# pytorch/ao

Measured on AMD Instinct MI355X. Metric: linear-layer tokens/sec, Llama-3-8B int4-wo (tinygemm g128), bs=1, higher is better.
Workload: dtype bf16 x int4 (dequant bf16, fp32 accumulate); 1 GPU; Int4WeightOnlyConfig(group_size=128) Llama-3-8B linear shapes, bs=1 seq=1, 32 layers x {qkv 6144x4096, o 4096x4096, gate 14336x4096, up 14336x4096, down 4096x14336}; module_layout=SURVEY.md 8(d) five shapes (qkv merged; gate, up separate), launch=hipGraph replay, parallelism=dp1 (one token stream per GPU, no collective)

## Files before the change

ao_amd/_lib.py:

```python
import ctypes
import os
import re
import threading

_HERE = os.path.dirname(os.path.abspath(__file__))
LIB_PATH = os.environ.get("AO_MI355_LIB") or os.path.join(_HERE, "_C_mi355.so")
HEADER_PATH = os.path.join(os.path.dirname(_HERE), "include", "ao_mi355.h")

AO_OK = 0
AO_ERR_INVALID_ARGUMENT = -1
AO_ERR_NULL_POINTER = -2
AO_ERR_HIP = -3

_lock = threading.Lock()
_lib = None

_P = ctypes.c_void_p
_I64 = ctypes.c_int64
_INT = ctypes.c_int

_SIGNATURES = {
    "ao_abi_version": [],
    "ao_prof_enable": [_INT],
    "ao_prof_collect": [_P, _INT, _P],
    "ao_splitk_reserve": [_P, _I64],
    "ao_splitk_query": [_P, _P],
    "ao_int4_convert_weight_to_int4pack": [_P, _P, _I64, _I64, _INT, _P],
    "ao_int4_unpack_int4pack": [_P, _P, _I64, _I64, _INT, _P],
    "ao_int4_weight_int4pack_mm": [_P, _P, _P, _P, _I64, _I64, _I64, _INT, _P],
    "ao_int4_weight_int4pack_mm_pair": [_P, _P, _P, _P, _P, _P, _P, _P, _I64, _I64, _I64, _INT, _P],
    "ao_int4_pair_independent": [_P, _P, _P, _P, _I64, _I64, _I64],
    "ao_int4_pair_fusions": [],
    "ao_int4_dequantize": [_P, _P, _P, _I64, _I64, _INT, _P],
    "ao_int4_quantize_tinygemm": [_P, _P, _P, _I64, _I64, _INT, _P],
    "ao_int4_hqq_workspace_bytes": [_I64, _I64, _INT],
    "ao_int4_quantize_hqq": [_P, _P, _P, _P, _I64, _I64, _INT, _P],
    "ao_int4_plain_quantize": [_P, _P, _P, _P, _I64, _I64, _INT, _INT, _P],
    "ao_int4_set_tuning": [_INT, _INT],
    "ao_int4_set_trace": [_P],
    "ao_gemm8_set_variant": [_INT],
    "ao_gemm8_set_tuning": [_INT, _INT],
    "ao_int4_mm_kernel_name": [_I64, _I64, _I64, _INT],
    "ao_gemm8_kernel_name": [_INT, _I64, _I64, _I64],
    "ao_fp8_int4_kernel_name": [_I64, _I64, _I64, _INT],
    "ao_gemm8_plan": [_INT, _I64, _I64, _I64, _P, _P],
    "ao_gemm8_plan_rows": [_INT, _I64, _I64, _I64, _P],
    "ao_gemm8_route": [_INT, _I64, _I64, _I64, _INT, _P, _INT],
# ... 157 lines not shown
            l.ao_fp8_block_grouped_mm_kernel_name.restype = ctypes.c_char_p
        if hasattr(l, "ao_nvfp4_linear_kernel_name"):
            l.ao_nvfp4_linear_kernel_name.restype = ctypes.c_char_p
        if hasattr(l, "ao_nvfp4_grouped_mm_kernel_name"):
            l.ao_nvfp4_grouped_mm_kernel_name.restype = ctypes.c_char_p
        if hasattr(l, "ao_fp8_int4_kernel_name"):
            l.ao_fp8_int4_kernel_name.restype = ctypes.c_char_p
        l.ao_moe_padded_rows.restype = _I64
        l.ao_mx_blocked_rows.restype = _I64
        l.ao_allreduce_flag_bytes.restype = _I64
        l.ao_allreduce_state_bytes.restype = _I64
        if hasattr(l, "ao_moe_a2a_flag_bytes"):
            l.ao_moe_a2a_flag_bytes.restype = _I64
            l.ao_moe_a2a_state_bytes.restype = _I64
        l.ao_int4_hqq_workspace_bytes.restype = _I64
        _lib = l
    return _lib


def last_error():
    return lib().ao_last_error().decode("utf-8", "replace")


def check(rc):
    if rc == AO_OK:
        return
    msg = last_error()
    if rc == AO_ERR_INVALID_ARGUMENT:
        raise ValueError(msg)
    raise RuntimeError(msg)
# ... 1 lines not shown
```

ao_amd/csrc/int4_kernels.hip:

```cpp
#include <algorithm>
#include <mutex>
#include <type_traits>
#include <utility>

#include "common.h"
#include "lds_dma.h"
#include "splitk.h"

namespace ao {
void fp8_rowwise_rb_set_trace(unsigned long long* p);
namespace {

__device__ __forceinline__ void dequant_word(uint32_t p, float s, float neg8s, float z,
                                             uint32_t (&out)[4]) {
  uint32_t lo = p & 0x0F0F0F0Fu;
  uint32_t hi = (p >> 4) & 0x0F0F0F0Fu;
  asm("" : "+v"(lo));
  asm("" : "+v"(hi));
  const float f0 = (float)(lo & 0xffu), f4 = (float)((lo >> 8) & 0xffu);
  const float f1 = (float)((lo >> 16) & 0xffu), f5 = (float)(lo >> 24);
  const float f2 = (float)(hi & 0xffu), f6 = (float)((hi >> 8) & 0xffu);
  const float f3 = (float)((hi >> 16) & 0xffu), f7 = (float)(hi >> 24);
  const f32x2 q[4] = {{f0, f1}, {f2, f3}, {f4, f5}, {f6, f7}};
#pragma unroll
// ... 68 lines not shown
    d.w0 = widen_add(ident, d.tp0, d.tp1, zz);
    d.w1 = widen_add(ident, d.tp2, d.tp3, zz);
#endif
  } else {
    d.out[0] = pack_bf16x2(d.w0.x, d.w0.y); d.out[1] = pack_bf16x2(d.w0.z, d.w0.w);
    d.out[2] = pack_bf16x2(d.w1.x, d.w1.y); d.out[3] = pack_bf16x2(d.w1.z, d.w1.w);
  }
}

template <int MAXM>
struct XRegs {
  static constexpr int kDwords = (MAXM <= 4) ? MAXM : MAXM;
  uint32_t v[kDwords];
};

template <int G, int MAXM, int DEPTH, bool STRAIGHT, bool BAL, bool STAMP>
__device__ __forceinline__ void int4_mm_body(
    const uint16_t* __restrict__ x, const u32x4* __restrict__ qdata,
    const uint32_t* __restrict__ sz, uint16_t* __restrict__ y, int M, int N, int K, float* __restrict__ ws, unsigned* __restrict__ tickets,
    const unsigned bx, const unsigned nbx) {
  static_assert(!(BAL || STAMP) || (STRAIGHT && MAXM == 1 && DEPTH == 4), "the balanced grid and the stamps exist on the 8 x 4 straight-line form");
  unsigned long long stamp[6] = {0, 0, 0, 0, 0, 0};
  if constexpr (STAMP) { stamp[0] = __builtin_amdgcn_s_memrealtime(); stamp[2] = __builtin_amdgcn_s_memtime(); }
  constexpr int NG = (G >= 128) ? 1 : (128 / G);
  constexpr int ROWSTRIDE = (MAXM <= 4) ? 256 : 272;
  constexpr int SLAB = (MAXM + 1) * ROWSTRIDE;
  extern __shared__ __attribute__((aligned(16))) char smem[];

  const int lane = threadIdx.x & 63;
  const int wave = __builtin_amdgcn_readfirstlane(threadIdx.x >> 6);
  const int nwaves = blockDim.x >> 6;
  int ntile = (int)bx;
  int kwave = wave;
  int part = -1;
  const int halves = BAL ? 2 * ((int)nbx - (N >> 4)) : 0;
  if constexpr (BAL) {
// ... 62 lines not shown
      }
    } else {
#pragma unroll
      for (int i = 0; i < MAXM / 4; ++i) {
        const int rr = min((lane >> 4) + 4 * i, last_row);
        const u32x4 t = *reinterpret_cast<const u32x4*>(xrow0 + (size_t)rr * K + kb * 128 + (lane & 15) * 8);
        s.xr.v[4 * i + 0] = t.x; s.xr.v[4 * i + 1] = t.y;
        s.xr.v[4 * i + 2] = t.z; s.xr.v[4 * i + 3] = t.w;
      }
    }
  };

  f32x4 acc = {0.f, 0.f, 0.f, 0.f};
  const s16x4 ident = identity_fragment(lane);

  auto stage_x = [&](const Stage& s, char* dst) {
    if (MAXM <= 4) {
#pragma unroll
      for (int r = 0; r < MAXM; ++r)
        *reinterpret_cast<uint32_t*>(dst + r * ROWSTRIDE + st_off) = s.xr.v[r];
    } else {
#pragma unroll
      for (int i = 0; i < MAXM / 4; ++i) {
        const int r = (lane >> 4) + 4 * i;
        char* d = dst + r * ROWSTRIDE + st_off;
        *reinterpret_cast<u32x2*>(d) = u32x2{s.xr.v[4 * i + 0], s.xr.v[4 * i + 1]};
        *reinterpret_cast<u32x2*>(d + 64) = u32x2{s.xr.v[4 * i + 2], s.xr.v[4 * i + 3]};
      }
    }
  };
// ... 19 lines not shown
    }
  };

  const int kb_last = max(kb1 - 1, kb0);
#pragma unroll
  for (int d = 0; d < DEPTH; ++d) issue(st[d], kFixedRun ? kb0 + d : min(kb0 + d, kb_last));

  auto for_slots = [&](auto&& f) {
    [&]<int... D>(std::integer_sequence<int, D...>) { (f(std::integral_constant<int, D>{}), ...); }(std::make_integer_sequence<int, DEPTH>{});
  };
  if constexpr (STRAIGHT) {
    if constexpr (STAMP) {
      asm volatile("s_waitcnt vmcnt(%0)" ::"n"(NG + 1 + (DEPTH - 1) * (NG + 2)) : "memory");
      stamp[3] = __builtin_amdgcn_s_memtime();
    }
    for_slots([&](auto dc) {
      constexpr int d = decltype(dc)::value;
      consume(st[d]);
    });
    if constexpr (STAMP) {
      asm volatile("" ::"v"(acc));
      stamp[4] = __builtin_amdgcn_s_memtime();
    }
    float* r = red + wave * 256 + (kq * 4) * 16 + (lane & 15);
    r[0] = acc.x; r[16] = acc.y; r[32] = acc.z; r[48] = acc.w;
    acc = f32x4{0.f, 0.f, 0.f, 0.f};
  } else {
  int kb = kb0;
  for (; kb + 2 * DEPTH <= kb1; kb += DEPTH) {
    for_slots([&](auto dc) {
      constexpr int d = decltype(dc)::value;
      consume(st[d]);
// ... 49 lines not shown
          if (t == 1u) __hip_atomic_store(&tickets[pair], 0u, __ATOMIC_RELAXED, __HIP_MEMORY_SCOPE_AGENT);
        }
        t = __builtin_amdgcn_readfirstlane(t);
        if (t == 1u && lane < 16) {
          float other[4];
#pragma unroll
          for (int w = 0; w < 4; ++w)
            other[w] = __builtin_bit_cast(float, __builtin_amdgcn_raw_buffer_load_b32(rws, ((1 - part) * 64 + w * 16 + lane) * 4, 0, kSc1));
          float sum = 0.f;
#pragma unroll
          for (int w = 0; w < 8; ++w) sum += ((w >> 2) == part) ? red[(w & 3) * 256 + lane] : other[w & 3];
          y[(size_t)ntile * 16 + lane] = f32_to_bf16_bits(sum);
        }
      }
      write_stamps();
      return;
    }
  }
  const int row = tid >> 4, col = tid & 15;
  if (tid < 256 && row < rows) {
    float sum = 0.f;
    for (int w = 0; w < nwaves; ++w) sum += red[w * 256 + tid];
    y[(size_t)(m0 + row) * N + ntile * 16 + col] = f32_to_bf16_bits(sum);
  }
  write_stamps();
}

template <int G, int MAXM, int DEPTH, bool STRAIGHT = false, bool BAL = false, bool STAMP = false>
__global__ __launch_bounds__((MAXM > 4) ? 512 : 1024) void int4_mm_kernel(
    const uint16_t* __restrict__ x, const u32x4* __restrict__ qdata,
    const uint32_t* __restrict__ sz, uint16_t* __restrict__ y, int M, int N, int K, float* __restrict__ ws, unsigned* __restrict__ tickets) {
  int4_mm_body<G, MAXM, DEPTH, STRAIGHT, BAL, STAMP>(x, qdata, sz, y, M, N, K, ws, tickets, blockIdx.x, gridDim.x);
}

struct Int4PairArgs {
  const uint16_t* x0; const uint16_t* x1;
  const u32x4* q0; const u32x4* q1;
  const uint32_t* sz0; const uint32_t* sz1;
  uint16_t* y0; uint16_t* y1;
  int N, K;
  float* ws;
  unsigned* tickets;
};
template <int G, int DEPTH, bool BAL>
__global__ __launch_bounds__(1024) void int4_mm_pair_kernel(const Int4PairArgs a) {
  const bool second = blockIdx.z != 0;
  const int halves = BAL ? (int)gridDim.x - (a.N >> 4) : 0;
  int4_mm_body<G, 1, DEPTH, true, BAL, false>(second ? a.x1 : a.x0, second ? a.q1 : a.q0, second ? a.sz1 : a.sz0, second ? a.y1 : a.y0, 1, a.N, a.K,
                                              a.ws + (second ? (size_t)halves * 128 : 0), a.tickets + (second ? halves : 0), blockIdx.x, gridDim.x);
}

constexpr int kRbStages = 3;
constexpr int kRbWeightStages = 3;
constexpr int rb_wstages(int waves, int mt, int wst) {
  const int room = (160 * 1024 - kRbStages * mt * 4096) / (waves * wst);
  return room >= kRbWeightStages ? kRbWeightStages : (room < 3 ? 3 : room);
}

template <int G, int WAVES, int NT, int MT = 8, int ABL = 0, bool PROD = false>
__global__ __launch_bounds__(64 * WAVES * (PROD ? 2 : 1), (WAVES == 4 && !PROD) ? 2 : 1) void int4_mm_rb_kernel(
    const uint16_t* __restrict__ x, const u32x4* __restrict__ qdata, const uint32_t* __restrict__ sz, uint16_t* __restrict__ y, int M,
    int N, int K, float* __restrict__ ws, unsigned* __restrict__ tickets, unsigned long long* __restrict__ trace) {
  unsigned long long ts[13] = {0, 0, 0, 0, 0, 0, 0, 0, 0, 0, 0, 0, 0};
  if (ABL == 5) ts[0] = __builtin_amdgcn_s_memtime();
// ... 886 lines not shown
  }
  std::lock_guard<std::mutex> lock(mu);
  if (cached[dev] == 0) {
    int n = 0;
    if (hipDeviceGetAttribute(&n, hipDeviceAttributeMultiprocessorCount, dev) != hipSuccess || n <= 0) {
      (void)hipGetLastError();
      n = 256;
    }
    cached[dev] = n;
  }
  return cached[dev];
}

constexpr int kBalOff = 981, kBalOn = 982, kStampGrid = 983, kStampBal = 984;
constexpr int kPairOff = 985, kPairHalves = 986;

Int4Route int4_route(int64_t M, int64_t N, int64_t K, int G, const Int4Force& f) {
  Int4Route r;
  const bool bal_mode = (f.mode >= kBalOff && f.mode <= kStampBal) || f.mode == kPairOff || f.mode == kPairHalves;
  if (f.mode != 0 && !bal_mode) r = int4_forced_route(M, N, K, G, f);
  else if (M <= 16 && !(M > 8 && (N >> 4) >= 288) && !(M > 4 && (N >> 4) >= 1024)) r = tile_route(M, N, K);
  else if (w32_band(M, N)) r = w32_route(M, N, K, G);
  else r = rb_route(M, N, K, (M <= 16) ? 1 : (M <= 32) ? 2 : (M <= 64) ? 4 : 8);
  r.wpb = f.wpb;
  if ((f.mode == 0 || bal_mode) && r.form == Int4Route::Tile && r.rows == 1 && r.straight && r.depth == 4 && (K >> 7) == 32) {
    const bool forced = f.mode == kBalOn || f.mode == kStampBal;
    if (f.mode != kBalOff && f.mode != kStampGrid) r.halves = ao_int4_balanced_halves(N >> 4, device_cus(), forced);
    r.stamp = (f.mode == kStampGrid || f.mode == kStampBal) && G == 128;
  }
  return r;
}

#define AO_MM_ARGS x, qdata, sz, y, M, N, K

template <int G>
int launch_route(const Int4Route& r, const uint16_t* x, const int32_t* qdata, const uint16_t* sz, uint16_t* y, int64_t M, int64_t N, int64_t K,
                 hipStream_t stream) {
  const int s = r.split;
  switch (r.form) {
// ... 157 lines not shown

int launch_pair(int group_size, const PairGeom& g, const Int4Problem& a, const Int4Problem& b, int64_t N, int64_t K, hipStream_t stream) {
  float* ws = nullptr;
  unsigned* tickets = nullptr;
  if (g.halves > 0)
    if (int rc = splitk_workspace(stream, &ws, &tickets, (size_t)2 * g.halves * 128, 2)) return rc;
  const Int4PairArgs args = pair_args(a, b, N, K, ws, tickets);
  return with_pair_kernel(group_size, g.depth, g.halves > 0, [&](auto kern) {
    if (int rc = ensure_dynamic_lds(reinterpret_cast<const void*>(kern), g.smem, "hipFuncSetAttribute(int4_mm_pair_kernel)")) return rc;
    ao::launch(kern, g.grid, g.block, g.smem, stream, args);
    AO_LAUNCH_CHECK("int4_mm_pair_kernel launch");
    return (int)AO_OK;
  });
}

struct Capture {
  bool active = false;
  unsigned long long id = 0;
  const hipGraphNode_t* deps = nullptr;
  size_t ndeps = 0;
};
Capture capture_of(hipStream_t s) {
  Capture c;
  hipStreamCaptureStatus st = hipStreamCaptureStatusNone;
  hipGraph_t graph = nullptr;
  if (hipStreamGetCaptureInfo_v2(s, &st, &c.id, &graph, &c.deps, &c.ndeps) != hipSuccess) {
    (void)hipGetLastError();
    return Capture{};
  }
  c.active = st == hipStreamCaptureStatusActive;
  return c;
}

struct PairRecord {
  bool live = false, paired = false;
  unsigned long long id = 0;
  hipStream_t stream = nullptr;
  hipGraphNode_t node = nullptr;
  int group_size = 0, depth = 0, halves = 0;
  int64_t N = 0, K = 0;
  Int4Problem p{};
};
std::mutex g_pair_mu;
PairRecord g_pair;
long long g_pair_fusions = 0;

bool try_fuse_pair(const Capture& cap, hipStream_t stream, const Int4Route& r, int group_size, int64_t N, int64_t K, const Int4Problem& b, bool keep_halves) {
  std::lock_guard<std::mutex> lock(g_pair_mu);
  PairRecord& rec = g_pair;
  if (!rec.live) return false;
  if (rec.id != cap.id) {
    rec = PairRecord{};
    return false;
  }
  if (rec.paired || rec.stream != stream || cap.ndeps != 1 || cap.deps == nullptr || cap.deps[0] != rec.node) return false;
  if (rec.group_size != group_size || rec.N != N || rec.K != K || rec.depth != r.depth || rec.halves != r.halves) return false;
  if (!ao_int4_pair_independent(rec.p.x, rec.p.y, b.x, b.y, 1, N, K)) return false;
  PairGeom g;
  if (!pair_geometry(r, 1, N, K, keep_halves, &g)) return false;
  float* ws = nullptr;
  unsigned* tickets = nullptr;
  if (g.halves > 0 && !splitk_workspace_held(stream, &ws, &tickets, (size_t)2 * g.halves * 128)) return false;
  Int4PairArgs args = pair_args(rec.p, b, N, K, ws, tickets);
  const hipGraphNode_t node = rec.node;
  const int rc = with_pair_kernel(group_size, g.depth, g.halves > 0, [&](auto kern) {
    void* params[1] = {&args};
    hipKernelNodeParams np{};
    np.func = reinterpret_cast<void*>(kern);
    np.gridDim = g.grid;
    np.blockDim = g.block;
    np.sharedMemBytes = (unsigned)g.smem;
    np.kernelParams = params;
    np.extra = nullptr;
    const hipError_t e = hipGraphKernelNodeSetParams(node, &np);
    if (e != hipSuccess) {
      (void)hipGetLastError();
      set_error("int4 pair fusion: hipGraphKernelNodeSetParams refused the pair kernel: %s (%s); launched on its own", hipGetErrorString(e), hipGetErrorName(e));
      return (int)AO_ERR_HIP;
    }
    return (int)AO_OK;
  });
  if (rc != AO_OK) {
    rec = PairRecord{};
    return false;
  }
  rec.paired = true;
  ++g_pair_fusions;
  return true;
}

void record_pair_candidate(const Capture& before, hipStream_t stream, const Int4Route& r, int group_size, int64_t N, int64_t K, const Int4Problem& p) {
  const Capture now = capture_of(stream);
  hipGraphNodeType type = hipGraphNodeTypeCount;
  const bool ok = now.active && now.id == before.id && now.ndeps == 1 && now.deps != nullptr &&
                  hipGraphNodeGetType(now.deps[0], &type) == hipSuccess && type == hipGraphNodeTypeKernel;
  if (!ok) (void)hipGetLastError();
  std::lock_guard<std::mutex> lock(g_pair_mu);
  g_pair = PairRecord{};
  if (!ok) return;
  g_pair.live = true;
  g_pair.id = now.id;
  g_pair.stream = stream;
  g_pair.node = now.deps[0];
  g_pair.group_size = group_size; g_pair.depth = r.depth; g_pair.halves = r.halves;
  g_pair.N = N; g_pair.K = K;
  g_pair.p = p;
}

}
}

using namespace ao;

extern "C" int ao_int4_balanced_halves(int64_t tiles, int cus, int forced) {
  if (tiles <= 0 || cus <= 0) return 0;
  const int64_t r = tiles % cus;
  if (r > kSplitMaxTickets) return 0;
  if (forced) return (int)r;
  return (tiles > cus && tiles <= 4ll * cus && 2 * r == cus) ? (int)r : 0;
}

// ... 69 lines not shown
extern "C" int ao_int4_weight_int4pack_mm(const uint16_t* x, const int32_t* qdata,
                                          const uint16_t* scale_and_zero, uint16_t* y, int64_t M,
                                          int64_t N, int64_t K, int group_size, void* stream) {
  AO_REQUIRE_PTR(qdata);
  AO_REQUIRE_PTR(scale_and_zero);
  if (int rc = check_int4_shape(__func__, N, K, group_size)) return rc;
  AO_REQUIRE(M >= 0 && M < (1ll << 31), "ao_int4_weight_int4pack_mm: bad M=%lld", (long long)M);
  if (M == 0) return AO_OK;
  AO_REQUIRE_PTR(x);
  AO_REQUIRE_PTR(y);
  hipStream_t s = (hipStream_t)stream;
  Capture cap;
  Int4Route twin;
  bool candidate = false;
  const Int4Problem prob{x, qdata, scale_and_zero, y};
  if (M == 1 && (cap = capture_of(s)).active) {
    PairGeom g;
    twin = int4_route(M, N, K, group_size, g_int4_force);
    candidate = pair_geometry(twin, M, N, K, true, &g);
    if (candidate && g_int4_force.mode != kPairOff && try_fuse_pair(cap, s, twin, group_size, N, K, prob, g_int4_force.mode == kPairHalves))
      return AO_OK;
  }
  const int64_t by_bytes = ((1ll << 32) - 1) / (2 * K) / 128 * 128;
  const int64_t chunk = std::max<int64_t>(128, std::min<int64_t>(by_bytes, 65535ll * 16));
  for (int64_t m0 = 0; m0 < M; m0 += chunk) {
    const int64_t rows = std::min(chunk, M - m0);
    const uint16_t* xc = x + m0 * K;
    uint16_t* yc = y + m0 * N;
    int rc;
    switch (group_size) {
      case 32: rc = dispatch_mm<32>(xc, qdata, scale_and_zero, yc, rows, N, K, s); break;
      case 64: rc = dispatch_mm<64>(xc, qdata, scale_and_zero, yc, rows, N, K, s); break;
      case 128: rc = dispatch_mm<128>(xc, qdata, scale_and_zero, yc, rows, N, K, s); break;
      default: rc = dispatch_mm<256>(xc, qdata, scale_and_zero, yc, rows, N, K, s); break;
    }
    if (rc != AO_OK) return rc;
  }
  if (candidate) record_pair_candidate(cap, s, twin, group_size, N, K, prob);
  return AO_OK;
}

extern "C" int ao_int4_pair_independent(const uint16_t* x0, const uint16_t* y0, const uint16_t* x1, const uint16_t* y1, int64_t M, int64_t N,
                                        int64_t K) {
  if (M <= 0 || N <= 0 || K <= 0) return 0;
  const auto overlap = [](const uint16_t* a, int64_t na, const uint16_t* b, int64_t nb) {
    const uintptr_t a0 = reinterpret_cast<uintptr_t>(a), b0 = reinterpret_cast<uintptr_t>(b);
    return a0 < b0 + 2 * (uintptr_t)nb && b0 < a0 + 2 * (uintptr_t)na;
  };
  return !overlap(y1, M * N, x0, M * K) && !overlap(y1, M * N, y0, M * N) && !overlap(x1, M * K, y0, M * N);
}

extern "C" int ao_int4_pair_fusions(void) {
  std::lock_guard<std::mutex> lock(g_pair_mu);
  return (int)std::min<long long>(g_pair_fusions, 0x7fffffff);
}

extern "C" int ao_int4_weight_int4pack_mm_pair(const uint16_t* x0, const int32_t* q0, const uint16_t* sz0, uint16_t* y0, const uint16_t* x1,
                                               const int32_t* q1, const uint16_t* sz1, uint16_t* y1, int64_t M, int64_t N, int64_t K,
                                               int group_size, void* stream) {
  AO_REQUIRE_PTR(q0);
  AO_REQUIRE_PTR(sz0);
  AO_REQUIRE_PTR(q1);
  AO_REQUIRE_PTR(sz1);
  if (int rc = check_int4_shape(__func__, N, K, group_size)) return rc;
  AO_REQUIRE(M >= 0 && M < (1ll << 31), "ao_int4_weight_int4pack_mm_pair: bad M=%lld", (long long)M);
  if (M == 0) return AO_OK;
  AO_REQUIRE_PTR(x0);
  AO_REQUIRE_PTR(y0);
  AO_REQUIRE_PTR(x1);
  AO_REQUIRE_PTR(y1);
  PairGeom g;
  const Int4Force& f = g_int4_force;
  if (M == 1 && ao_int4_pair_independent(x0, y0, x1, y1, M, N, K) &&
      pair_geometry(int4_route(M, N, K, group_size, f), M, N, K, f.mode == kPairHalves, &g))
    return launch_pair(group_size, g, Int4Problem{x0, q0, sz0, y0}, Int4Problem{x1, q1, sz1, y1}, N, K, (hipStream_t)stream);
  if (int rc = ao_int4_weight_int4pack_mm(x0, q0, sz0, y0, M, N, K, group_size, stream)) return rc;
  return ao_int4_weight_int4pack_mm(x1, q1, sz1, y1, M, N, K, group_size, stream);
}

extern "C" int ao_int4_dequantize(const int32_t* qdata, const uint16_t* scale_and_zero,
                                  uint16_t* w_bf16, int64_t N, int64_t K, int group_size,
                                  void* stream) {
  AO_REQUIRE_PTR(qdata);
  AO_REQUIRE_PTR(scale_and_zero);
  AO_REQUIRE_PTR(w_bf16);
  if (int rc = check_int4_shape(__func__, N, K, group_size)) return rc;
  const int64_t words = N * K / 8;
  const int threads = 256;
  dim3 grid((unsigned)((words + threads - 1) / threads)), block(threads);
  const uint32_t* q = reinterpret_cast<const uint32_t*>(qdata);
// ... 35 lines not shown
```

ao_amd/ops.py:

```python
import ctypes
from typing import Optional

import torch

from . import _lib

__all__ = [
    "convert_weight_to_int4pack",
    "unpack_int4pack",
    "weight_int4pack_mm",
    "int4_dequantize",
    "int4_quantize_tinygemm",
    "int4_plain_quantize",
    "int4_quantize_hqq",
    "int8_quantize_rowwise",
    "int8_scaled_mm",
    "int_mm",
    "fp8_quantize_rowwise",
    "fp8_scaled_mm",
    "mxfp8_quantize",
    "mxfp8_grouped_mm",
    "mxfp8_grouped_mm_wgrad",
    "mxfp8_mm_wgrad",
    "dynamic_linear_fits",
# ... 166 lines not shown
    m = x0.shape[0]
    y0 = torch.empty((m, n), dtype=torch.bfloat16, device=dev)
    y1 = torch.empty((m, n), dtype=torch.bfloat16, device=dev)
    if m == 0:
        return y0, y1
    with _on(dev):
        _lib.check(
            _lib.lib().ao_int4_weight_int4pack_mm_pair(
                _ptr(x0), _ptr(qdata0), _ptr(scale_and_zero0), _ptr(y0), _ptr(x1), _ptr(qdata1), _ptr(scale_and_zero1), _ptr(y1),
                m, n, k, group_size, _stream()
            )
        )
    return y0, y1


def int4_dequantize(qdata: torch.Tensor, scale_and_zero: torch.Tensor, group_size: int) -> torch.Tensor:
    dev = _require_gpu("int4_dequantize", qdata, scale_and_zero)
    n, k = _int4_dims("int4_dequantize", qdata, scale_and_zero, group_size)
    w = torch.empty((n, k), dtype=torch.bfloat16, device=dev)
    with _on(dev):
        _lib.check(
            _lib.lib().ao_int4_dequantize(_ptr(qdata), _ptr(scale_and_zero), _ptr(w), n, k, group_size, _stream())
        )
    return w


def int4_quantize_tinygemm(w: torch.Tensor, group_size: int):
    dev = _require_gpu("int4_quantize_tinygemm", w)
    if w.dim() != 2 or w.dtype != torch.bfloat16:
        raise RuntimeError("int4_quantize_tinygemm: expected a 2-D bfloat16 tensor")
# ... 1844 lines not shown
```

include/ao_mi355.h:

```cpp
#ifndef AO_MI355_H
#define AO_MI355_H

#include <stddef.h>
#include <stdint.h>

#ifdef __cplusplus
extern "C" {
#endif

#define AO_OK 0
#define AO_ERR_INVALID_ARGUMENT (-1)
#define AO_ERR_NULL_POINTER (-2)
#define AO_ERR_HIP (-3)

#define AO_MI355_ABI_VERSION 2

int ao_abi_version(void);
const char* ao_last_error(void);

int ao_splitk_reserve(void* stream, int64_t bytes);

int ao_splitk_query(void* stream, int64_t out_host[4]);

int ao_prof_enable(int max_records);
// ... 6 lines not shown

int ao_int4_unpack_int4pack(const int32_t* qdata, uint8_t* w_u8, int64_t N,
                            int64_t K, int inner_k_tiles, void* stream);

int ao_int4_weight_int4pack_mm(const uint16_t* x, const int32_t* qdata,
                               const uint16_t* scale_and_zero, uint16_t* y,
                               int64_t M, int64_t N, int64_t K, int group_size,
                               void* stream);

int ao_int4_weight_int4pack_mm_pair(const uint16_t* x0, const int32_t* qdata0, const uint16_t* scale_and_zero0, uint16_t* y0,
                                    const uint16_t* x1, const int32_t* qdata1, const uint16_t* scale_and_zero1, uint16_t* y1,
                                    int64_t M, int64_t N, int64_t K, int group_size, void* stream);
int ao_int4_pair_independent(const uint16_t* x0, const uint16_t* y0, const uint16_t* x1, const uint16_t* y1, int64_t M, int64_t N,
                             int64_t K);
int ao_int4_pair_fusions(void);

int ao_int4_dequantize(const int32_t* qdata, const uint16_t* scale_and_zero,
                       uint16_t* w_bf16, int64_t N, int64_t K, int group_size,
                       void* stream);

int ao_int4_quantize_tinygemm(const uint16_t* w, int32_t* qdata,
                              uint16_t* scale_and_zero, int64_t N, int64_t K,
                              int group_size, void* stream);

int ao_int4_set_tuning(int waves_per_block, int mode);
int ao_int4_overridden(void);
int ao_gemm8_set_variant(int variant);
int ao_gemm8_set_tuning(int key, int value);
int ao_gemm8_overridden(void);
const char* ao_int4_mm_kernel_name(int64_t M, int64_t N, int64_t K, int group_size);
// ... 293 lines not shown
```

Measured before the change: 944.0 tokens/s.

## Prefetch the next layer's int4 weights into cache from the current GEMV

Adds an optional prefetch hint: each wave of the one-row straight-line int4 GEMV kernel issues one buffer load, spread over a span of the next packed weight tensor, so those lines are warm in cache when the next kernel starts. The hint can be set explicitly per stream, or patched into an already captured graph node, including a fused pair kernel. The goal is to hide the next GEMV's DRAM start-up latency behind the current kernel. In exchange the kernel issues extra memory traffic that competes for bandwidth, and the change adds host bookkeeping, a pointer-range validation and graph-node parameter rewrites.

```diff
diff --git a/ao_amd/_lib.py b/ao_amd/_lib.py
--- a/ao_amd/_lib.py
+++ b/ao_amd/_lib.py
@@ -31,6 +31,9 @@
     "ao_int4_weight_int4pack_mm_pair": [_P, _P, _P, _P, _P, _P, _P, _P, _I64, _I64, _I64, _INT, _P],
     "ao_int4_pair_independent": [_P, _P, _P, _P, _I64, _I64, _I64],
     "ao_int4_pair_fusions": [],
+    "ao_int4_set_prefetch_hint": [_P, ctypes.c_size_t, _P],
+    "ao_int4_prefetch_hints": [],
+    "ao_int4_prefetch_span": [_I64, _I64, _INT, _INT, _INT, _INT, _INT, ctypes.c_uint64, ctypes.c_uint64, _P, _I64],
     "ao_int4_dequantize": [_P, _P, _P, _I64, _I64, _INT, _P],
     "ao_int4_quantize_tinygemm": [_P, _P, _P, _I64, _I64, _INT, _P],
     "ao_int4_hqq_workspace_bytes": [_I64, _I64, _INT],
@@ -218,6 +221,8 @@
             l.ao_moe_a2a_flag_bytes.restype = _I64
             l.ao_moe_a2a_state_bytes.restype = _I64
         l.ao_int4_hqq_workspace_bytes.restype = _I64
+        if hasattr(l, "ao_int4_prefetch_span"):
+            l.ao_int4_prefetch_span.restype = _I64
         _lib = l
     return _lib
 
diff --git a/ao_amd/csrc/int4_kernels.hip b/ao_amd/csrc/int4_kernels.hip
--- a/ao_amd/csrc/int4_kernels.hip
+++ b/ao_amd/csrc/int4_kernels.hip
@@ -1,9 +1,12 @@
 #include <algorithm>
+#include <atomic>
 #include <mutex>
 #include <type_traits>
 #include <utility>
+#include <vector>
 
 #include "common.h"
+#include "int4_prefetch.h"
 #include "lds_dma.h"
 #include "splitk.h"
 
@@ -106,12 +109,13 @@
   uint32_t v[kDwords];
 };
 
-template <int G, int MAXM, int DEPTH, bool STRAIGHT, bool BAL, bool STAMP>
+template <int G, int MAXM, int DEPTH, bool STRAIGHT, bool BAL, bool STAMP, int PF = 0>
 __device__ __forceinline__ void int4_mm_body(
     const uint16_t* __restrict__ x, const u32x4* __restrict__ qdata,
     const uint32_t* __restrict__ sz, uint16_t* __restrict__ y, int M, int N, int K, float* __restrict__ ws, unsigned* __restrict__ tickets,
-    const unsigned bx, const unsigned nbx) {
+    const unsigned bx, const unsigned nbx, const Int4Pf pf = Int4Pf{}, const unsigned bz = 0) {
   static_assert(!(BAL || STAMP) || (STRAIGHT && MAXM == 1 && DEPTH == 4), "the balanced grid and the stamps exist on the 8 x 4 straight-line form");
+  static_assert(PF == 0 || (STRAIGHT && MAXM == 1 && !STAMP), "the prefetch hint exists on the one-row straight-line forms");
   unsigned long long stamp[6] = {0, 0, 0, 0, 0, 0};
   if constexpr (STAMP) { stamp[0] = __builtin_amdgcn_s_memrealtime(); stamp[2] = __builtin_amdgcn_s_memtime(); }
   constexpr int NG = (G >= 128) ? 1 : (128 / G);
@@ -204,6 +208,20 @@
   f32x4 acc = {0.f, 0.f, 0.f, 0.f};
   const s16x4 ident = identity_fragment(lane);
 
+  uint32_t pf_back = 0;
+  auto prefetch = [&] {
+    if constexpr (PF != 0) {
+      const __amdgpu_buffer_rsrc_t rp = __builtin_amdgcn_make_buffer_rsrc(const_cast<void*>(pf.base), 0, (int)pf.bytes, 0x00020000);
+      const uint32_t gw = int4_pf_wave(bx, bz, (uint32_t)wave, nbx, (uint32_t)nwaves, (uint32_t)halves);
+      if constexpr (PF == 2) __builtin_amdgcn_sched_barrier(0);
+      pf_back = __builtin_amdgcn_raw_buffer_load_b32(rp, (int)int4_pf_offset(gw, (uint32_t)lane, pf.shift, pf.period), 0, 0);
+      if constexpr (PF == 2) __builtin_amdgcn_sched_barrier(0);
+    }
+  };
+  auto prefetch_done = [&] {
+    if constexpr (PF != 0) asm volatile("" ::"v"(pf_back));
+  };
+
   auto stage_x = [&](const Stage& s, char* dst) {
     if (MAXM <= 4) {
 #pragma unroll
@@ -253,8 +271,10 @@
       asm volatile("s_waitcnt vmcnt(%0)" ::"n"(NG + 1 + (DEPTH - 1) * (NG + 2)) : "memory");
       stamp[3] = __builtin_amdgcn_s_memtime();
     }
+    if constexpr (PF == 1) prefetch();
     for_slots([&](auto dc) {
       constexpr int d = decltype(dc)::value;
+      if constexpr (PF == 2 && d == DEPTH - 1) prefetch();
       consume(st[d]);
     });
     if constexpr (STAMP) {
@@ -334,6 +354,7 @@
         }
       }
       write_stamps();
+      prefetch_done();
       return;
     }
   }
@@ -344,6 +365,7 @@
     y[(size_t)(m0 + row) * N + ntile * 16 + col] = f32_to_bf16_bits(sum);
   }
   write_stamps();
+  prefetch_done();
 }
 
 template <int G, int MAXM, int DEPTH, bool STRAIGHT = false, bool BAL = false, bool STAMP = false>
@@ -351,6 +373,14 @@
     const uint16_t* __restrict__ x, const u32x4* __restrict__ qdata,
     const uint32_t* __restrict__ sz, uint16_t* __restrict__ y, int M, int N, int K, float* __restrict__ ws, unsigned* __restrict__ tickets) {
   int4_mm_body<G, MAXM, DEPTH, STRAIGHT, BAL, STAMP>(x, qdata, sz, y, M, N, K, ws, tickets, blockIdx.x, gridDim.x);
+}
+
+template <int G, int DEPTH, bool BAL, int PF>
+__global__ __launch_bounds__(1024) void int4_mm_pf_kernel(
+    const uint16_t* __restrict__ x, const u32x4* __restrict__ qdata,
+    const uint32_t* __restrict__ sz, uint16_t* __restrict__ y, int M, int N, int K, float* __restrict__ ws, unsigned* __restrict__ tickets,
+    const Int4Pf pf) {
+  int4_mm_body<G, 1, DEPTH, true, BAL, false, PF>(x, qdata, sz, y, M, N, K, ws, tickets, blockIdx.x, gridDim.x, pf, 0);
 }
 
 struct Int4PairArgs {
@@ -368,6 +398,19 @@
   const int halves = BAL ? (int)gridDim.x - (a.N >> 4) : 0;
   int4_mm_body<G, 1, DEPTH, true, BAL, false>(second ? a.x1 : a.x0, second ? a.q1 : a.q0, second ? a.sz1 : a.sz0, second ? a.y1 : a.y0, 1, a.N, a.K,
                                               a.ws + (second ? (size_t)halves * 128 : 0), a.tickets + (second ? halves : 0), blockIdx.x, gridDim.x);
+}
+struct Int4PairPfArgs {
+  Int4PairArgs a;
+  Int4Pf pf;
+};
+template <int G, int DEPTH, bool BAL, int PF>
+__global__ __launch_bounds__(1024) void int4_mm_pair_pf_kernel(const Int4PairPfArgs p) {
+  const Int4PairArgs& a = p.a;
+  const bool second = blockIdx.z != 0;
+  const int halves = BAL ? (int)gridDim.x - (a.N >> 4) : 0;
+  int4_mm_body<G, 1, DEPTH, true, BAL, false, PF>(second ? a.x1 : a.x0, second ? a.q1 : a.q0, second ? a.sz1 : a.sz0, second ? a.y1 : a.y0, 1, a.N, a.K,
+                                                  a.ws + (second ? (size_t)halves * 128 : 0), a.tickets + (second ? halves : 0), blockIdx.x, gridDim.x,
+                                                  p.pf, blockIdx.z);
 }
 
 constexpr int kRbStages = 3;
@@ -1284,15 +1327,27 @@
 
 constexpr int kBalOff = 981, kBalOn = 982, kStampGrid = 983, kStampBal = 984;
 constexpr int kPairOff = 985, kPairHalves = 986;
+constexpr int kPfOff = 987, kPfFirst0 = 988, kPfLast2 = 993;
+struct PfPlan {
+  int point = 0;
+  int run = 0;
+};
+constexpr PfPlan kPfProductAuto = {0, 0}, kPfProductExplicit = {2, 0};
+PfPlan pf_plan(int mode, bool explicit_hint) {
+  if (mode == kPfOff) return PfPlan{};
+  if (mode >= kPfFirst0 && mode <= kPfLast2) return PfPlan{mode <= 990 ? 1 : 2, ((mode - kPfFirst0) % 3 == 2) ? 0 : (mode - kPfFirst0) % 3 + 1};
+  return explicit_hint ? kPfProductExplicit : kPfProductAuto;
+}
 
 Int4Route int4_route(int64_t M, int64_t N, int64_t K, int G, const Int4Force& f) {
   Int4Route r;
-  const bool bal_mode = (f.mode >= kBalOff && f.mode <= kStampBal) || f.mode == kPairOff || f.mode == kPairHalves;
+  const bool pf_mode = f.mode >= kPfOff && f.mode <= kPfLast2;
+  const bool bal_mode = (f.mode >= kBalOff && f.mode <= kStampBal) || f.mode == kPairOff || f.mode == kPairHalves || pf_mode;
   if (f.mode != 0 && !bal_mode) r = int4_forced_route(M, N, K, G, f);
   else if (M <= 16 && !(M > 8 && (N >> 4) >= 288) && !(M > 4 && (N >> 4) >= 1024)) r = tile_route(M, N, K);
   else if (w32_band(M, N)) r = w32_route(M, N, K, G);
   else r = rb_route(M, N, K, (M <= 16) ? 1 : (M <= 32) ? 2 : (M <= 64) ? 4 : 8);
-  r.wpb = f.wpb;
+  r.wpb = pf_mode ? 0 : f.wpb;
   if ((f.mode == 0 || bal_mode) && r.form == Int4Route::Tile && r.rows == 1 && r.straight && r.depth == 4 && (K >> 7) == 32) {
     const bool forced = f.mode == kBalOn || f.mode == kStampBal;
     if (f.mode != kBalOff && f.mode != kStampGrid) r.halves = ao_int4_balanced_halves(N >> 4, device_cus(), forced);
@@ -1480,6 +1535,129 @@
   });
 }
 
+struct PfTarget {
+  const void* q = nullptr;
+  uint64_t bytes = 0;
+  int blocks_per_wave = 0;
+};
+
+Int4Pf pf_span(const PfPlan& plan, const PfTarget& t, uint64_t waves) {
+  Int4Pf pf;
+  if (plan.point == 0 || t.q == nullptr || t.bytes == 0 || waves == 0) return pf;
+  const bool strided = plan.run > 0 && t.blocks_per_wave > plan.run;
+  pf.shift = (strided && plan.run == 2) ? 4u : 3u;
+  pf.period = strided ? 1024u * (uint32_t)t.blocks_per_wave : (kPfLine << pf.shift);
+  if (int4_pf_max_offset(waves, pf.shift, pf.period) >= (1ull << 32)) return pf;
+  pf.base = t.q;
+  pf.bytes = (uint32_t)std::min<uint64_t>(t.bytes, 0xffffff80ull);
+  return pf;
+}
+
+template <typename F>
+int with_pf_kernels(int group_size, int depth, bool bal, int point, F&& f) {
+  auto on_g = [&](auto gc) {
+    constexpr int G = decltype(gc)::value;
+    auto on_d = [&](auto dc, auto bc) {
+      constexpr int D = decltype(dc)::value;
+      constexpr bool B = decltype(bc)::value;
+      return point == 1 ? f(int4_mm_pf_kernel<G, D, B, 1>, int4_mm_pair_pf_kernel<G, D, B, 1>) : f(int4_mm_pf_kernel<G, D, B, 2>, int4_mm_pair_pf_kernel<G, D, B, 2>);
+    };
+    using std::integral_constant;
+    switch (depth) {
+      case 4: return bal ? on_d(integral_constant<int, 4>{}, std::true_type{}) : on_d(integral_constant<int, 4>{}, std::false_type{});
+      case 7: return on_d(integral_constant<int, 7>{}, std::false_type{});
+      case 14: return on_d(integral_constant<int, 14>{}, std::false_type{});
+      case 2: return on_d(integral_constant<int, 2>{}, std::false_type{});
+      case 8: return on_d(integral_constant<int, 8>{}, std::false_type{});
+      case 9: return on_d(integral_constant<int, 9>{}, std::false_type{});
+    }
+    set_error("int4_mm (hinted): no %d-deep kernel", depth);
+    return (int)AO_ERR_INVALID_ARGUMENT;
+  };
+  switch (group_size) {
+    case 32: return on_g(std::integral_constant<int, 32>{});
+    case 64: return on_g(std::integral_constant<int, 64>{});
+    case 128: return on_g(std::integral_constant<int, 128>{});
+    default: return on_g(std::integral_constant<int, 256>{});
+  }
+}
+
+struct HintedLaunch {
+  int group_size = 0, point = 0;
+  PairGeom g;
+  Int4Problem a{}, b{};
+  int64_t N = 0, K = 0;
+  float* ws = nullptr;
+  unsigned* tickets = nullptr;
+  Int4Pf pf;
+};
+uint64_t live_waves(const PairGeom& g) {
+  return (uint64_t)g.grid.z * int4_pf_live_waves(g.grid.x, g.block.x / 64, 2u * (unsigned)g.halves);
+}
+
+int hinted_launch(const HintedLaunch& h, hipStream_t stream, hipGraphNode_t node) {
+  return with_pf_kernels(h.group_size, h.g.depth, h.g.halves > 0, h.point, [&](auto single, auto pair) {
+    const bool two = h.g.grid.z == 2;
+    const void* func = two ? reinterpret_cast<const void*>(pair) : reinterpret_cast<const void*>(single);
+    const uint16_t* x = h.a.x;
+    const u32x4* q = reinterpret_cast<const u32x4*>(h.a.q);
+    const uint32_t* sz = reinterpret_cast<const uint32_t*>(h.a.sz);
+    uint16_t* y = h.a.y;
+    int M = 1, N = (int)h.N, K = (int)h.K;
+    float* ws = h.ws;
+    unsigned* tickets = h.tickets;
+    Int4Pf pf = h.pf;
+    Int4PairPfArgs pargs{pair_args(h.a, h.b, h.N, h.K, h.ws, h.tickets), h.pf};
+    if (node != nullptr) {
+      void* one[10] = {&x, &q, &sz, &y, &M, &N, &K, &ws, &tickets, &pf};
+      void* both[1] = {&pargs};
+      hipKernelNodeParams np{};
+      np.func = const_cast<void*>(func);
+      np.gridDim = h.g.grid;
+      np.blockDim = h.g.block;
+      np.sharedMemBytes = (unsigned)h.g.smem;
+      np.kernelParams = two ? both : one;
+      np.extra = nullptr;
+      const hipError_t e = hipGraphKernelNodeSetParams(node, &np);
+      if (e != hipSuccess) {
+        (void)hipGetLastError();
+        set_error("int4 prefetch hint: hipGraphKernelNodeSetParams refused the hinted kernel: %s (%s); the launch stays as it was", hipGetErrorString(e),
+                  hipGetErrorName(e));
+        return (int)AO_ERR_HIP;
+      }
+      return (int)AO_OK;
+    }
+    if (int rc = ensure_dynamic_lds(func, h.g.smem, "hipFuncSetAttribute(int4_mm_pf_kernel)")) return rc;
+    if (two) ao::launch(pair, h.g.grid, h.g.block, h.g.smem, stream, pargs);
+    else ao::launch(single, h.g.grid, h.g.block, h.g.smem, stream, x, q, sz, y, M, N, K, ws, tickets, pf);
+    AO_LAUNCH_CHECK("int4_mm_pf_kernel launch");
+    return (int)AO_OK;
+  });
+}
+
+std::mutex g_pf_mu;
+struct PfPending {
+  hipStream_t stream;
+  PfTarget t;
+};
+std::vector<PfPending> g_pf_pending;
+std::atomic<int> g_pf_pending_n{0};
+std::atomic<long long> g_pf_hints{0};
+
+PfTarget take_explicit_hint(hipStream_t s) {
+  PfTarget t;
+  if (g_pf_pending_n.load(std::memory_order_acquire) == 0) return t;
+  std::lock_guard<std::mutex> lock(g_pf_mu);
+  for (size_t i = 0; i < g_pf_pending.size(); ++i)
+    if (g_pf_pending[i].stream == s) {
+      t = g_pf_pending[i].t;
+      g_pf_pending.erase(g_pf_pending.begin() + (long)i);
+      g_pf_pending_n.store((int)g_pf_pending.size(), std::memory_order_release);
+      break;
+    }
+  return t;
+}
+
 struct Capture {
   bool active = false;
   unsigned long long id = 0;
@@ -1505,13 +1683,17 @@
   hipGraphNode_t node = nullptr;
   int group_size = 0, depth = 0, halves = 0;
   int64_t N = 0, K = 0;
-  Int4Problem p{};
+  Int4Problem p{}, p2{};
+  int pair_halves = 0;
+  PfPlan hint_plan{};
+  PfTarget hint{};
 };
 std::mutex g_pair_mu;
 PairRecord g_pair;
 long long g_pair_fusions = 0;
 
-bool try_fuse_pair(const Capture& cap, hipStream_t stream, const Int4Route& r, int group_size, int64_t N, int64_t K, const Int4Problem& b, bool keep_halves) {
+bool try_fuse_pair(const Capture& cap, hipStream_t stream, const Int4Route& r, int group_size, int64_t N, int64_t K, const Int4Problem& b, bool keep_halves,
+                   const PfPlan& plan_b, const PfTarget& hint_b) {
   std::lock_guard<std::mutex> lock(g_pair_mu);
   PairRecord& rec = g_pair;
   if (!rec.live) return false;
@@ -1529,7 +1711,13 @@
   if (g.halves > 0 && !splitk_workspace_held(stream, &ws, &tickets, (size_t)2 * g.halves * 128)) return false;
   Int4PairArgs args = pair_args(rec.p, b, N, K, ws, tickets);
   const hipGraphNode_t node = rec.node;
-  const int rc = with_pair_kernel(group_size, g.depth, g.halves > 0, [&](auto kern) {
+  const PfPlan plan = plan_b.point != 0 ? plan_b : rec.hint_plan;
+  const PfTarget hint = plan_b.point != 0 ? hint_b : rec.hint;
+  HintedLaunch h;
+  h.group_size = group_size; h.point = plan.point; h.g = g; h.a = rec.p; h.b = b; h.N = N; h.K = K; h.ws = ws; h.tickets = tickets;
+  h.pf = pf_span(plan, hint, live_waves(g));
+  const bool hinted = h.pf.bytes != 0;
+  const int rc = hinted ? hinted_launch(h, stream, node) : with_pair_kernel(group_size, g.depth, g.halves > 0, [&](auto kern) {
     void* params[1] = {&args};
     hipKernelNodeParams np{};
     np.func = reinterpret_cast<void*>(kern);
@@ -1551,11 +1739,61 @@
     return false;
   }
   rec.paired = true;
+  rec.p2 = b;
+  rec.pair_halves = g.halves;
+  if (rec.hint_plan.point != 0 && !hinted) g_pf_hints.fetch_sub(1);
+  if (rec.hint_plan.point == 0 && hinted) g_pf_hints.fetch_add(1);
+  rec.hint_plan = hinted ? plan : PfPlan{};
+  rec.hint = hinted ? hint : PfTarget{};
   ++g_pair_fusions;
   return true;
 }
 
-void record_pair_candidate(const Capture& before, hipStream_t stream, const Int4Route& r, int group_size, int64_t N, int64_t K, const Int4Problem& p) {
+bool pf_target_live(const PfTarget& t) {
+  hipPointerAttribute_t attr{};
+  if (hipPointerGetAttributes(&attr, t.q) != hipSuccess || attr.type != hipMemoryTypeDevice) {
+    (void)hipGetLastError();
+    return false;
+  }
+  hipDeviceptr_t base = nullptr;
+  size_t size = 0;
+  if (hipMemGetAddressRange(&base, &size, const_cast<void*>(t.q)) != hipSuccess) {
+    (void)hipGetLastError();
+    return false;
+  }
+  const uintptr_t b0 = reinterpret_cast<uintptr_t>(base), q0 = reinterpret_cast<uintptr_t>(t.q);
+  return q0 >= b0 && t.bytes <= size && q0 - b0 <= size - t.bytes;
+}
+
+bool try_hint_recorded(const Capture& cap, const PfPlan& plan, const PfTarget& t) {
+  if (plan.point == 0) return false;
+  std::lock_guard<std::mutex> lock(g_pair_mu);
+  PairRecord& rec = g_pair;
+  if (!rec.live) return false;
+  if (rec.id != cap.id) {
+    rec = PairRecord{};
+    return false;
+  }
+  if (rec.hint_plan.point != 0) return false;
+  if (!pf_target_live(t)) return false;
+  Int4Route r = tile_form(1, rec.depth, true);
+  r.halves = rec.paired ? rec.pair_halves : rec.halves;
+  HintedLaunch h;
+  if (!pair_geometry(r, 1, rec.N, rec.K, true, &h.g)) return false;
+  if (!rec.paired) h.g.grid.z = 1;
+  if (h.g.halves > 0 && !splitk_workspace_held(rec.stream, &h.ws, &h.tickets, (size_t)h.g.grid.z * h.g.halves * 128)) return false;
+  h.group_size = rec.group_size; h.point = plan.point; h.a = rec.p; h.b = rec.p2; h.N = rec.N; h.K = rec.K;
+  h.pf = pf_span(plan, t, live_waves(h.g));
+  if (h.pf.bytes == 0) return false;
+  if (hinted_launch(h, rec.stream, rec.node) != AO_OK) return false;
+  rec.hint_plan = plan;
+  rec.hint = t;
+  g_pf_hints.fetch_add(1);
+  return true;
+}
+
+void record_pair_candidate(const Capture& before, hipStream_t stream, const Int4Route& r, int group_size, int64_t N, int64_t K, const Int4Problem& p,
+                           const PfPlan& hint_plan, const PfTarget& hint) {
   const Capture now = capture_of(stream);
   hipGraphNodeType type = hipGraphNodeTypeCount;
   const bool ok = now.active && now.id == before.id && now.ndeps == 1 && now.deps != nullptr &&
@@ -1571,6 +1809,8 @@
   g_pair.group_size = group_size; g_pair.depth = r.depth; g_pair.halves = r.halves;
   g_pair.N = N; g_pair.K = K;
   g_pair.p = p;
+  g_pair.hint_plan = hint_plan;
+  g_pair.hint = hint;
 }
 
 }
@@ -1670,12 +1910,36 @@
   Int4Route twin;
   bool candidate = false;
   const Int4Problem prob{x, qdata, scale_and_zero, y};
-  if (M == 1 && (cap = capture_of(s)).active) {
-    PairGeom g;
+  const PfTarget hint = take_explicit_hint(s);
+  const PfPlan hint_plan = hint.bytes != 0 ? pf_plan(g_int4_force.mode, true) : PfPlan{};
+  PairGeom g;
+  if (M == 1 && ((cap = capture_of(s)).active || hint_plan.point != 0)) {
     twin = int4_route(M, N, K, group_size, g_int4_force);
     candidate = pair_geometry(twin, M, N, K, true, &g);
-    if (candidate && g_int4_force.mode != kPairOff && try_fuse_pair(cap, s, twin, group_size, N, K, prob, g_int4_force.mode == kPairHalves))
+    if (cap.active && candidate && g_int4_force.mode != kPairOff &&
+        try_fuse_pair(cap, s, twin, group_size, N, K, prob, g_int4_force.mode == kPairHalves, hint_plan, hint))
       return AO_OK;
+  }
+  if (cap.active) {
+    PfTarget mine;
+    mine.q = qdata;
+    mine.bytes = (uint64_t)N * (uint64_t)K / 2;
+    mine.blocks_per_wave = candidate ? twin.depth : 0;
+    (void)try_hint_recorded(cap, pf_plan(g_int4_force.mode, false), mine);
+  }
+  if (candidate && hint_plan.point != 0) {
+    HintedLaunch h;
+    g.grid.z = 1;
+    h.group_size = group_size; h.point = hint_plan.point; h.g = g; h.a = prob; h.N = N; h.K = K;
+    h.pf = pf_span(hint_plan, hint, live_waves(g));
+    if (h.pf.bytes != 0) {
+      if (g.halves > 0)
+        if (int rc = splitk_workspace(s, &h.ws, &h.tickets, (size_t)g.halves * 128, 2)) return rc;
+      if (int rc = hinted_launch(h, s, nullptr)) return rc;
+      g_pf_hints.fetch_add(1);
+      if (cap.active) record_pair_candidate(cap, s, twin, group_size, N, K, prob, hint_plan, hint);
+      return AO_OK;
+    }
   }
   const int64_t by_bytes = ((1ll << 32) - 1) / (2 * K) / 128 * 128;
   const int64_t chunk = std::max<int64_t>(128, std::min<int64_t>(by_bytes, 65535ll * 16));
@@ -1692,7 +1956,7 @@
     }
     if (rc != AO_OK) return rc;
   }
-  if (candidate) record_pair_candidate(cap, s, twin, group_size, N, K, prob);
+  if (candidate && cap.active) record_pair_candidate(cap, s, twin, group_size, N, K, prob, PfPlan{}, PfTarget{});
   return AO_OK;
 }
 
@@ -1709,6 +1973,61 @@
 extern "C" int ao_int4_pair_fusions(void) {
   std::lock_guard<std::mutex> lock(g_pair_mu);
   return (int)std::min<long long>(g_pair_fusions, 0x7fffffff);
+}
+
+extern "C" int ao_int4_set_prefetch_hint(const void* qdata, size_t bytes, void* stream) {
+  AO_REQUIRE_PTR(qdata);
+  AO_REQUIRE(reinterpret_cast<uintptr_t>(qdata) % 16 == 0, "ao_int4_set_prefetch_hint: qdata must be 16-byte aligned (a packed weight's first block)");
+  PfPending e;
+  e.stream = (hipStream_t)stream;
+  e.t.q = qdata;
+  e.t.bytes = bytes;
+  const Int4Force& f = g_int4_force;
+  e.t.blocks_per_wave = (f.mode >= kPfFirst0 && f.mode <= kPfLast2) ? f.wpb : 0;
+  std::lock_guard<std::mutex> lock(g_pf_mu);
+  for (size_t i = 0; i < g_pf_pending.size(); ++i)
+    if (g_pf_pending[i].stream == e.stream) g_pf_pending.erase(g_pf_pending.begin() + (long)i--);
+  if (bytes != 0) g_pf_pending.push_back(e);
+  g_pf_pending_n.store((int)g_pf_pending.size(), std::memory_order_release);
+  return AO_OK;
+}
+
+extern "C" int ao_int4_prefetch_hints(void) { return (int)std::min<long long>(g_pf_hints.load(), 0x7fffffff); }
+
+extern "C" int64_t ao_int4_prefetch_span(int64_t N, int64_t K, int group_size, int pair, int halved_tiles, int run, int period_blocks, uint64_t bytes,
+                                         uint64_t cap, uint32_t* out, int64_t out_cap) {
+  if (check_int4_shape(__func__, N, K, group_size) != AO_OK || group_size == 0) return -1;
+  Int4Route r = int4_route(1, N, K, group_size, Int4Force{});
+  r.halves = halved_tiles;
+  PairGeom g;
+  if (run < 0 || run > 2 || period_blocks < 0 || halved_tiles < 0 || halved_tiles > (N >> 4) || (halved_tiles > 0 && r.depth != 4) ||
+      !pair_geometry(r, 1, N, K, true, &g)) {
+    set_error("ao_int4_prefetch_span: no one-row straight-line launch for N=%lld K=%lld (halved tiles %d, run %d, period %d)", (long long)N, (long long)K,
+              halved_tiles, run, period_blocks);
+    return -1;
+  }
+  if (!pair) g.grid.z = 1;
+  PfTarget t;
+  t.q = &t;
+  t.bytes = std::min(bytes, cap);
+  t.blocks_per_wave = period_blocks;
+  const PfPlan plan{1, run};
+  const Int4Pf pf = pf_span(plan, t, live_waves(g));
+  int64_t n = 0;
+  if (pf.bytes == 0) return 0;
+  const unsigned nwaves = g.block.x / 64, half_wgs = 2u * (unsigned)g.halves;
+  for (unsigned bz = 0; bz < g.grid.z; ++bz)
+    for (unsigned bx = 0; bx < g.grid.x; ++bx)
+      for (unsigned w = 0; w < (bx < half_wgs ? 4u : nwaves); ++w) {
+        const uint32_t gw = int4_pf_wave(bx, bz, w, g.grid.x, nwaves, half_wgs);
+        for (unsigned lane = 0; lane < 64; ++lane) {
+          const uint32_t off = int4_pf_offset(gw, lane, pf.shift, pf.period);
+          if (!int4_pf_touched(off, pf.bytes)) continue;
+          if (out != nullptr && n < out_cap) out[n] = off;
+          ++n;
+        }
+      }
+  return n;
 }
 
 extern "C" int ao_int4_weight_int4pack_mm_pair(const uint16_t* x0, const int32_t* q0, const uint16_t* sz0, uint16_t* y0, const uint16_t* x1,
@@ -1728,8 +2047,21 @@
   PairGeom g;
   const Int4Force& f = g_int4_force;
   if (M == 1 && ao_int4_pair_independent(x0, y0, x1, y1, M, N, K) &&
-      pair_geometry(int4_route(M, N, K, group_size, f), M, N, K, f.mode == kPairHalves, &g))
+      pair_geometry(int4_route(M, N, K, group_size, f), M, N, K, f.mode == kPairHalves, &g)) {
+    const PfTarget hint = take_explicit_hint((hipStream_t)stream);
+    HintedLaunch h;
+    h.point = hint.bytes != 0 ? pf_plan(f.mode, true).point : 0;
+    if (h.point != 0) h.pf = pf_span(pf_plan(f.mode, true), hint, live_waves(g));
+    if (h.pf.bytes != 0) {
+      h.group_size = group_size; h.g = g; h.a = Int4Problem{x0, q0, sz0, y0}; h.b = Int4Problem{x1, q1, sz1, y1}; h.N = N; h.K = K;
+      if (g.halves > 0)
+        if (int rc = splitk_workspace((hipStream_t)stream, &h.ws, &h.tickets, (size_t)2 * g.halves * 128, 2)) return rc;
+      if (int rc = hinted_launch(h, (hipStream_t)stream, nullptr)) return rc;
+      g_pf_hints.fetch_add(1);
+      return AO_OK;
+    }
     return launch_pair(group_size, g, Int4Problem{x0, q0, sz0, y0}, Int4Problem{x1, q1, sz1, y1}, N, K, (hipStream_t)stream);
+  }
   if (int rc = ao_int4_weight_int4pack_mm(x0, q0, sz0, y0, M, N, K, group_size, stream)) return rc;
   return ao_int4_weight_int4pack_mm(x1, q1, sz1, y1, M, N, K, group_size, stream);
 }
diff --git a/ao_amd/csrc/int4_prefetch.h b/ao_amd/csrc/int4_prefetch.h
--- /dev/null
+++ b/ao_amd/csrc/int4_prefetch.h
@@ -0,0 +1,35 @@
+#pragma once
+#include <stdint.h>
+
+namespace ao {
+
+struct Int4Pf {
+  const void* base = nullptr;
+  uint32_t bytes = 0;
+  uint32_t period = 1024;
+  uint32_t shift = 3;
+};
+
+constexpr uint32_t kPfLine = 128;
+
+__host__ __device__ inline uint32_t int4_pf_live_waves(uint32_t nbx, uint32_t nwaves, uint32_t half_wgs) {
+  return half_wgs * 4u + (nbx - half_wgs) * nwaves;
+}
+__host__ __device__ inline uint32_t int4_pf_wave(uint32_t bx, uint32_t bz, uint32_t wave, uint32_t nbx, uint32_t nwaves, uint32_t half_wgs) {
+  const uint32_t in_problem = bx < half_wgs ? bx * 4u + wave : half_wgs * 4u + (bx - half_wgs) * nwaves + wave;
+  return bz * int4_pf_live_waves(nbx, nwaves, half_wgs) + in_problem;
+}
+
+__host__ __device__ inline uint32_t int4_pf_offset(uint32_t gw, uint32_t lane, uint32_t shift, uint32_t period) {
+  const uint32_t wave_part = ((gw * 64u) >> shift) * period;
+  const uint32_t lane_part = (lane >> shift) * period + (lane & ((1u << shift) - 1u)) * kPfLine;
+  return wave_part + lane_part;
+}
+
+__host__ __device__ inline bool int4_pf_touched(uint32_t off, uint32_t bytes) { return (uint64_t)off + 4u <= bytes; }
+
+inline uint64_t int4_pf_max_offset(uint64_t waves, uint32_t shift, uint32_t period) {
+  return (((waves * 64u) >> shift) + 1u) * (uint64_t)period;
+}
+
+}
diff --git a/ao_amd/ops.py b/ao_amd/ops.py
--- a/ao_amd/ops.py
+++ b/ao_amd/ops.py
@@ -204,6 +204,22 @@
     return y0, y1
 
 
+def int4_prefetch_hint(qdata: torch.Tensor, nbytes: int = None) -> None:
+    dev = _require_gpu("int4_prefetch_hint", qdata)
+    if not qdata.is_contiguous():
+        raise RuntimeError("int4_prefetch_hint: qdata must be contiguous")
+    total = qdata.numel() * qdata.element_size()
+    nbytes = total if nbytes is None else int(nbytes)
+    if nbytes < 0 or nbytes > total:
+        raise RuntimeError(f"int4_prefetch_hint: nbytes={nbytes} outside the tensor's {total} bytes")
+    with _on(dev):
+        _lib.check(_lib.lib().ao_int4_set_prefetch_hint(_ptr(qdata), nbytes, _stream()))
+
+
+def int4_prefetch_hints() -> int:
+    return int(_lib.lib().ao_int4_prefetch_hints())
+
+
 def int4_dequantize(qdata: torch.Tensor, scale_and_zero: torch.Tensor, group_size: int) -> torch.Tensor:
     dev = _require_gpu("int4_dequantize", qdata, scale_and_zero)
     n, k = _int4_dims("int4_dequantize", qdata, scale_and_zero, group_size)
diff --git a/include/ao_mi355.h b/include/ao_mi355.h
--- a/include/ao_mi355.h
+++ b/include/ao_mi355.h
@@ -44,6 +44,11 @@
 int ao_int4_pair_independent(const uint16_t* x0, const uint16_t* y0, const uint16_t* x1, const uint16_t* y1, int64_t M, int64_t N,
                              int64_t K);
 int ao_int4_pair_fusions(void);
+
+int ao_int4_set_prefetch_hint(const void* qdata, size_t bytes, void* stream);
+int ao_int4_prefetch_hints(void);
+int64_t ao_int4_prefetch_span(int64_t N, int64_t K, int group_size, int pair, int halved_tiles, int run, int period_blocks, uint64_t bytes,
+                              uint64_t cap, uint32_t* out, int64_t out_cap);
 
 int ao_int4_dequantize(const int32_t* qdata, const uint16_t* scale_and_zero,
                        uint16_t* w_bf16, int64_t N, int64_t K, int group_size,
```

Measured after the change: 931.0 tokens/s. 0.986x the previous value.
